# tudoroancea/ihm2

Hardware: AMD Instinct MI355X
Metric: NMPC RTI solves/s (batch), N=40, nx=8 (6-DOF bicycle), fkin6 (higher is better)
Workload: dtype f64

## Files before the change

ihm2_amd/csrc/device_steps.hpp:

```cpp
#pragma once

#include "ihm2mpc_internal.h"
#include "model.hpp"
#include "rk4.hpp"

namespace ihm2 {

__device__ __forceinline__ void dev_prepare(int b, int lane, int N, double s_target, int mode, const double *x0,
                                            double *x, double *u, double *yref, double *yref_e)
{
    double *xb = x + (size_t)b * (N + 1) * 8, *ub = u + (size_t)b * N * 2;
    if (mode & 1) {
        const double s0 = x0[(size_t)b * 8];
        double *yb = yref + (size_t)b * N * 12, *ye = yref_e + (size_t)b * 8;
        for (int e = lane; e < N * 12; e += 64) yb[e] = (e % 12 == 0) ? s0 + s_target * (e / 12) / N : 0.0;
        if (lane < 8) ye[lane] = (lane == 0) ? s0 + s_target : 0.0;
    }
    if (!(mode & 2)) return;
    const int nx = N * 8;
    for (int base = 0; base < nx; base += 64) {
        const int e = base + lane;
        const double v = (e < nx) ? xb[e + 8] : 0.0;
        __syncthreads();
        if (e < nx) xb[e] = v;
        __syncthreads();
    }
    const int nu = N * 2;
    for (int base = 0; base < nu; base += 64) {
        const int e = base + lane;
        const double v = (e < nu - 2) ? ub[e + 2] : 0.0;
        __syncthreads();
        if (e < nu) ub[e] = v;
        __syncthreads();
    }
}

__device__ __forceinline__ void dev_wrap_lap(int b, int lane, int N, int nknots, const double *__restrict__ s_ref, const int32_t *__restrict__ track_id,
                                             double *x0, double *x)
{
    const double L = -s_ref[(size_t)track_id[b] * nknots];
    if (!(x0[(size_t)b * 8] >= L)) return;
    for (int k = lane; k <= N; k += 64) x[((size_t)b * (N + 1) + k) * 8] -= L;
    if (lane == 0) x0[(size_t)b * 8] -= L;
}

__host__ __device__ constexpr int s_pos(int mdl, int c, int i)
{
    int p = 0;
    for (int cc = 0; cc < c; cc++)
        for (int b = 0; b < 8; b++) p += (S_COL_MASK[mdl][cc] >> b) & 1u;
    for (int b = 0; b < i; b++) p += (S_COL_MASK[mdl][c] >> b) & 1u;
    return p;
}
__host__ __device__ constexpr int s_count(int mdl) { return s_pos(mdl, 10, 0); }

template <int COL>
__device__ __forceinline__ double fkin6_factored_row(int i, const double (&J)[8][10], const double (&dX)[8], const double (&dK)[8])
{
    constexpr unsigned cm = S_COL_MASK[0][COL];
    double acc = 0.0;
    if (i == 2) {
        if ((cm >> 5) & 1u) acc = dX[5];
        acc = fma(-J[FKIN6_F_ROW2][FKIN6_F_DKS], dX[0], acc);
        acc = fma(-J[FKIN6_F_ROW2][FKIN6_F_KAP], dK[0], acc);
    } else {
        if (COL == 9) acc = -J[FKIN6_F_ROW5][FKIN6_F_DBD_DU];
        if ((cm >> 4) & 1u) acc = fma(k_lR, dK[4], acc);
        if ((cm >> 7) & 1u) acc = fma(-J[FKIN6_F_ROW5][FKIN6_F_DBD_DD], dX[7], acc);
    }
    return acc;
}

template <int MODEL, int COL, bool FACTORED = false>
__device__ __forceinline__ void sens_col_stage(const double (&J)[8][10], const double (&S)[8], const double *Sl, double (&Sacc)[8],
                                               double (&dK)[8], double ah, double wh)
{
    static_assert(!FACTORED || MODEL == IHM2MPC_MODEL_FKIN6, "the factored Jacobian is fkin6's");
    constexpr unsigned cm = S_COL_MASK[MODEL ? 1 : 0][COL];
    double dX[8];
#pragma unroll
    for (int l = 0; l < 8; l++)
        if ((cm >> l) & 1u) dX[l] = fma(ah, dK[l], Sl ? Sl[s_pos(MODEL ? 1 : 0, COL, l) * 64] : S[l]);
#pragma unroll
    for (int i = 0; i < 8; i++) {
        if (!((cm >> i) & 1u)) continue;
        if (FACTORED && (i == 2 || i == 5)) { dK[i] = fkin6_factored_row<COL>(i, J, dX, dK); continue; }
        double acc = 0.0;
        if (COL >= 8 && ((JU_MASK[MODEL ? 1 : 0][i] >> (COL - 8)) & 1u)) acc = J[i][COL];
#pragma unroll
        for (int l = 0; l < 8; l++)
            if (((JX_MASK[MODEL ? 1 : 0][i] & cm) >> l) & 1u) acc = fma(J[i][l], dX[l], acc);
        dK[i] = acc;
    }
#pragma unroll
    for (int i = 0; i < 8; i++)
        if ((cm >> i) & 1u) Sacc[i] = fma(wh, dK[i], Sacc[i]);
}

template <int MODEL, int COL>
__device__ __forceinline__ void sens_col_copy(const double (&src)[8], double (&dst)[8])
{
    constexpr unsigned cm = S_COL_MASK[MODEL ? 1 : 0][COL];
#pragma unroll
    for (int i = 0; i < 8; i++)
        if ((cm >> i) & 1u) dst[i] = src[i];
}

template <int COL, bool FACTORED = false>
__device__ __forceinline__ void sens_col_stage_lag(const double (&J)[8][10], const double (&S)[8], double (&Sacc)[8], double (&dK)[8], double ah,
                                                   double wh, double E_T, double E_d)
{
    constexpr unsigned cm = S_COL_MASK[0][COL];
    double dX[8];
#pragma unroll
    for (int l = 0; l < 6; l++)
        if ((cm >> l) & 1u) dX[l] = fma(ah, dK[l], S[l]);
    if ((cm >> 6) & 1u) dX[6] = (COL == 8) ? fma(E_T, S[6], 1.0 - E_T) : E_T * S[6];
// ... 272 lines not shown
```

ihm2_amd/csrc/kernels_qp.hip:

```cpp
#include <cstring>

#include "ihm2mpc_internal.h"
#include "device_steps.hpp"
#include "sqp_body.hpp"
#include "irk_body.hpp"
#include "riccati_mfma.hpp"
#include "sens_body.hpp"
#include "qp_lds.hpp"
#include "qp_mrows.hpp"
#include "qp_reduce.hpp"
#include "qp_div.hpp"
#include "qp_catalogue.hpp"
#include "wave_sync.hpp"

using namespace ihm2;

namespace {

#define INF_BOUND 1e20
#ifndef RIC_RING
#define RIC_RING 4
#endif
#ifndef SWEEP_RING
#define SWEEP_RING 4
// ... 154 lines not shown
    constexpr bool HL = CLS.hl, CL = CLS.cl;
    static_assert(qp_factor_inside(qp_lds(40, CLS), 40, NCK) && qp_factor_inside(qp_lds(2, CLS), 2, NCK), "factor stage / block reductions leave their LDS");
    static_assert(qp_sweeps_inside(qp_lds(40, CLS), 40, LEAN != 0, SWEEP_RING, SWEEP_DL) && (LEAN == 0 || qp_sweeps_inside(qp_lds(2, CLS), 2, true, SWEEP_RING, SWEEP_DL)),
                  "the sweeps' unclamped LDS prefetch leaves the block (the earlier form does below N = 4: api.hip refuses those launches)");
    static_assert(NW <= 4, "qp_factor_inside checks the block reductions for four waves");
    static_assert(FULL == 0 || qp_full_zeroes_kept(qp_lds(NF > 0 ? NF : 2, CLS), NF > 0 ? NF : 2), "a store of the factor sweep reaches gam or cf: the full slot form zeroes them once per solve");
#define LEN(id) qp_lds_len(id, N, NS, CLS)
    double *z = sm, *gt = z + LEN(QP_Z), *pi = gt + LEN(QP_GT), *pv = pi + LEN(QP_PI), *rb = pv + LEN(QP_PV), *gam = rb + LEN(QP_RB), *cf = gam + LEN(QP_GAM), *dz = cf + LEN(QP_CF);
    double *kff = dz + LEN(QP_DZ), *Kl = kff + LEN(QP_KFF), *Ginv = Kl + LEN(QP_KL), *Prb = Ginv + LEN(QP_GINV), *tile = Prb + LEN(QP_PRB), *hc = tile + LEN(QP_TILE), *ha = hc + LEN(QP_HC);
    double *Hl = ha + LEN(QP_HA), *CDl = Hl + LEN(QP_HL), *spv = CDl + LEN(QP_CDL);
    int *spc = reinterpret_cast<int *>(spv + 60);
#undef LEN
#define HS(k, i, l) (HL ? Hl[(((k) == N) ? 100 : 0) + (i) * 10 + (l)] : ((k) == N ? HsT : Hs0 + (UNI ? 0 : (k)) * 100)[(i) * 10 + (l)])
#define CDV(k, r, j) (CL ? CDl[(r) * 10 + (j)] : a.CD[((k) * 2 + (r)) * 10 + (j)])

    auto blk_reduce = [&](double v, auto op) -> double {
        v = wave_reduce(v, op);
        if (NW > 1) {
            __syncthreads();
            if (lane == 0) tile[wv] = v;
            __syncthreads();
            v = tile[0];
#pragma unroll
            for (int w = 1; w < NW; w++) v = op(v, tile[w]);
        }
        return v;
    };
    auto blk_max = [&](double v) { return blk_reduce(v, [](double x, double y) { return fmax(x, y); }); };
    auto blk_min = [&](double v) { return blk_reduce(v, [](double x, double y) { return fmin(x, y); }); };
    auto blk_sum = [&](double v) { return blk_reduce(v, [](double x, double y) { return x + y; }); };
    auto blk_nanmax = [&](double v) { return blk_reduce(v, [](double x, double y) { return nanmax(x, y); }); };

    const double *xb = a.x + (size_t)b * NS * 8;
    const double *ub = a.u + (size_t)b * N * 2;
    const double *linb = a.lin + (size_t)b * N * LIN_REC;
    double *gb = a.g + (size_t)b * NS * 10;
    double *rgb = a.rg + (size_t)b * NS * 10;
    double *Pg = a.P + (size_t)b * NS * 64;
    double *Mg = a.M + (size_t)b * N * 64;
    double *pib = a.pi + (size_t)b * NS * 8;
    double *lamb = a.lam + (size_t)b * NS * 28;
    double *slkb = a.slk + (size_t)b * NS * 28;
    double *lamab = ALAT ? a.lam_a + (size_t)b * NS * 2 : nullptr;
    double *slkab = ALAT ? a.slk_a + (size_t)b * NS * 2 : nullptr;
    auto alat_slot = [](int j) -> int { return (j == 3) ? 0 : (j == 4) ? 1 : (j == 6) ? 2 : (j == 7) ? 3 : -1; };

    if (HL) for (int e = tid; e < 200; e += NT) Hl[e] = (e < 100) ? Hs0[e] : HsT[e - 100];
    if (CL && tid < 20) CDl[tid] = a.CD[tid];
    if (UNI) BSYNC();
    bool h_sparse = false;
    if (HL) {
        int cnt = 0;
        if (tid < 20) {
#pragma unroll
            for (int l = 0; l < 10; l++) {
                const double v = Hl[tid * 10 + l];
                if (v != 0.0) { if (cnt < 3) { spv[tid * 3 + cnt] = v; spc[tid * 3 + cnt] = l; } cnt++; }
            }
            for (int q = cnt; q < 3; q++) { spv[tid * 3 + q] = 0.0; spc[tid * 3 + q] = 0; }
        }
        h_sparse = __ballot(cnt > 3) == 0ull;
        if (NW > 1) h_sparse = blk_max((wv == 0 && !h_sparse) ? 1.0 : 0.0) == 0.0;
        BSYNC();
    }
    double sg = 1.0, sb = 1.0, r_stat = 0.0, r_eq = 0.0;
    double w_R = 0.0, w_L = 0.0;
    if (PATH) {
        const int trk = a.track_id[b];
        w_R = a.widths[trk * 2 + 0]; w_L = a.widths[trk * 2 + 1];
        for (int k = tid; k < NS; k += NT) {
            const double psi = xb[k * 8 + 2], sgn = (psi > 0.0) - (psi < 0.0);
            const double dfoot = -0.5 * a.car_L * cos(fabs(psi)) * sgn, dlat = -0.5 * a.car_W * sin(psi);
            hc[k * 2 + 0] = (k >= 1) ? dfoot + dlat : 0.0;
            hc[k * 2 + 1] = (k >= 1) ? -dfoot + dlat : 0.0;
            if (ALAT) {
                double g4[4];
                alat_eval(xb[k * 8 + 3], xb[k * 8 + 4], xb[k * 8 + 6], xb[k * 8 + 7], g4);
#pragma unroll
                for (int q = 0; q < 4; q++) ha[k * 4 + q] = (k >= 1 && k < N) ? g4[q] : 0.0;
            }
        }
        BSYNC();
    }
    for (int e = tid; e < NS * 10; e += NT) {
        const int k = e / 10, j = e % 10;
        double acc = 0.0;
#pragma unroll
        for (int l = 0; l < 8; l++) acc = fma(HS(k, j, l), xb[k * 8 + l], acc);
        if (k < N) {
            acc = fma(HS(k, j, 8), ub[k * 2 + 0], acc);
            acc = fma(HS(k, j, 9), ub[k * 2 + 1], acc);
            const double *yr = a.yref + ((size_t)b * N + k) * 12;
#pragma unroll
            for (int l = 0; l < 12; l++) acc = fma(-Gy0[((UNI ? 0 : k) * 10 + j) * 12 + l], yr[l], acc);
        } else {
            const double *yr = a.yref_e + (size_t)b * 8;
#pragma unroll
            for (int l = 0; l < 8; l++) acc = fma(-GyT[j * 12 + l], yr[l], acc);
        }
        gb[e] = acc;
        const bool counted = !((k == 0 && j < 8) || (k == N && j >= 8));
        if (j < 8 || k < N) sg = fmax(sg, fabs(acc));
        if (!want_res) continue;
        double st = acc;
        if (k < N) {
            const double *rec = linb + (size_t)k * LIN_REC;
#pragma unroll
            for (int l = 0; l < 8; l++) st = fma((j < 8) ? rec[l * 8 + j] : rec[64 + l * 2 + (j - 8)], pib[(k + 1) * 8 + l], st);
        }
        if (j < 8) st -= pib[k * 8 + j];
        st -= lamb[k * 28 + j] - lamb[k * 28 + 14 + j];
        if (k < N) {
            st = fma(-CDV(k, 0, j), lamb[k * 28 + 10] - lamb[k * 28 + 24], st);
            st = fma(-CDV(k, 1, j), lamb[k * 28 + 11] - lamb[k * 28 + 25], st);
        }
        if (PATH && (j == 1 || j == 2)) {
            const double l12 = lamb[k * 28 + 12] - lamb[k * 28 + 26], l13 = lamb[k * 28 + 13] - lamb[k * 28 + 27];
            st -= (j == 1) ? l12 - l13 : hc[k * 2] * l12 + hc[k * 2 + 1] * l13;
        }
        if (ALAT && alat_slot(j) >= 0) st -= ha[k * 4 + alat_slot(j)] * (lamab[k * 2] - lamab[k * 2 + 1]);
        if (counted) r_stat = fmax(r_stat, fabs(st));
    }
    for (int e = tid; e < N * 8; e += NT) {
        const double bl = linb[(size_t)(e / 8) * LIN_REC + 80 + (e % 8)];
        sb = fmax(sb, fabs(bl));
        r_eq = fmax(r_eq, fabs(bl));
    }
    if (tid < 8) {
        const double d = a.x0[(size_t)b * 8 + tid] - xb[tid];
        sb = fmax(sb, fabs(d));
        r_eq = fmax(r_eq, fabs(d));
    }
    if constexpr (FULL != 0) { double sg2 = sg, sb2 = sb; wave_max4(lane, sg, sb, sg2, sb2); }
    else { sg = blk_max(sg); sb = blk_max(sb); }

    int s_kc[NSLOT];
    double s_dl[NSLOT], s_du[NSLOT];
    double lam_l[NSLOT], lam_u[NSLOT], t_l[NSLOT], t_u[NSLOT];
    constexpr int NSO = (NSOFT > 0) ? NSOFT : 1;
    double so_zw[NSO], so_Zw[NSO], so_s[NSO], so_ls[NSO], so_rs[NSO], so_ds[NSO], so_dls[NSO], so_pa[NSO];
#pragma unroll
    for (int r = 0; r < NSO; r++) { so_zw[r] = 0.0; so_Zw[r] = -1.0; so_s[r] = 1.0; so_ls[r] = 0.0; so_rs[r] = 0.0; so_ds[r] = so_dls[r] = so_pa[r] = 0.0; }
#define IS_SOFT(r) ((r) < NSOFT && so_Zw[(r) < NSOFT ? (r) : 0] >= 0.0)
#define ONE_SIDED(r) (NSOFT > 0 && PATH != 2 && (r) < NSOFT)
#define HAS_L(r) (FULL ? true : ONE_SIDED(r) ? true : fin(s_dl[r]))
#define HAS_U(r) (FULL ? true : ONE_SIDED(r) ? false : fin(s_du[r]))
#define ROW_DOT(r, v) (FULL ? row_dot_full((r), (v)) : ONE_SIDED(r) ? s_sg[(r) < NSOFT ? (r) : 0] * row_dot(s_kc[r], (v)) : row_dot(s_kc[r], (v)))
#define NO_SLOT(r) (!FULL && s_kc[r] < 0)
#define SLOT_W(r) (FULL ? (s_kc[r] & 0xffff) >> 3 : s_kc[r])
#define SLOT_AT(arr, r) (*(FULL ? reinterpret_cast<double *>(reinterpret_cast<char *>(arr) + (here(s_kc[r]) & 0xffff)) : &(arr)[s_kc[r]]))
#define ROW_SIGN(r, c) (ONE_SIDED(r) ? s_sg[(r) < NSOFT ? (r) : 0] * (c) : (c))
    double s_sg[NSO];
#pragma unroll
    for (int r = 0; r < NSO; r++) s_sg[r] = 1.0;
#define SLOT_ACC(dst, v) do { if (NSOFT > 0) (dst) += (v); else (dst) = (v); } while (0)
    double r_ineq = 0.0, r_comp = 0.0;
#pragma unroll
    for (int r = 0; r < NSLOT; r++) {
        const int s = tid + NT * r;
        s_kc[r] = FULL ? 0 : -1; s_dl[r] = -INFINITY; s_du[r] = INFINITY;
        lam_l[r] = lam_u[r] = 0.0; t_l[r] = t_u[r] = 1.0;
        const int kc = (s < a.nslots) ? a.slot_kc[s] : -1;
        if (kc >= 0) {
            const int k = kc >> 4, c = kc & 15;
            s_kc[r] = k * NCK + c;
            if (FULL) s_kc[r] = qp_full_slot_pack(k, c, NCK);
            double cz;
            if (c < 8) cz = xb[k * 8 + c];
            else if (c < 10) cz = ub[k * 2 + c - 8];
            else if (ALAT && c == 14) {
                double g4[4];
                cz = alat_eval(xb[k * 8 + 3], xb[k * 8 + 4], xb[k * 8 + 6], xb[k * 8 + 7], g4);
            } else if (c >= 12) {
                const double n = xb[k * 8 + 1], psi = xb[k * 8 + 2];
                const double foot = -0.5 * a.car_L * sin(fabs(psi)), lat = 0.5 * a.car_W * cos(psi);
                cz = (c == 12) ? n + foot + lat - w_R : -n - foot + lat - w_L;
            } else {
                cz = 0.0;
#pragma unroll
                for (int j = 0; j < 8; j++) cz = fma(CDV(k, c - 10, j), xb[k * 8 + j], cz);
                cz = fma(CDV(k, c - 10, 8), ub[k * 2 + 0], cz);
                cz = fma(CDV(k, c - 10, 9), ub[k * 2 + 1], cz);
            }
            const double lb = slot_lbb[s], ubd = slot_ubb[s];
            bool soft = false;
            if (r < NSOFT) { so_zw[r < NSOFT ? r : 0] = a.slot_zw[s]; so_Zw[r < NSOFT ? r : 0] = a.slot_Zw[s]; soft = a.slot_Zw[s] >= 0.0; }
#define LAM_IN(up) ((ALAT && c == 14) ? lamab[k * 2 + (up)] : lamb[k * 28 + 14 * (up) + c])
            if (fin(lb)) { s_dl[r] = lb - cz; if (want_res && !soft) { r_ineq = fmax(r_ineq, s_dl[r]); r_comp = fmax(r_comp, fabs(LAM_IN(0) * s_dl[r])); } }
            if (fin(ubd)) { s_du[r] = ubd - cz; if (want_res && !soft) { r_ineq = fmax(r_ineq, -s_du[r]); r_comp = fmax(r_comp, fabs(LAM_IN(1) * s_du[r])); } }
#undef LAM_IN
            if (ONE_SIDED(r) && fin(ubd)) { s_sg[r < NSOFT ? r : 0] = -1.0; s_dl[r] = -s_du[r]; }
        }
    }
    if (want_res) {
        if constexpr (FULL != 0) wave_max4(lane, r_stat, r_eq, r_ineq, r_comp);
        else { r_stat = blk_max(r_stat); r_eq = blk_max(r_eq); r_ineq = blk_max(r_ineq); r_comp = blk_max(r_comp); }
    }
    if (want_res && tid == 0) {
        double *rs = a.res + (size_t)b * 4;
        rs[0] = r_stat; rs[1] = r_eq; rs[2] = r_ineq; rs[3] = r_comp;
    }

    const double tol_g = a.tol * sg, tol_b = a.tol * sb, tol_d = a.tol * sb, tol_m = a.tol * sg;
    const double mu_floor = 0.1 * tol_m;
    const double mu0 = a.mu0 * sg;
    const double inv_m = (a.m_act > 0) ? 1.0 / a.m_act : 0.0;

    auto row_dot = [&](int kc, const double *v) -> double {
        const int k = kc / NCK, c = kc % NCK;
        if (c < 10) return v[k * 10 + c];
        if (ALAT && c == 14) return ha[k * 4] * v[k * 10 + 3] + ha[k * 4 + 1] * v[k * 10 + 4] + ha[k * 4 + 2] * v[k * 10 + 6] + ha[k * 4 + 3] * v[k * 10 + 7];
        if (PATH && c >= 12) return (c == 12) ? v[k * 10 + 1] + hc[k * 2] * v[k * 10 + 2] : -v[k * 10 + 1] + hc[k * 2 + 1] * v[k * 10 + 2];
        double acc = 0.0;
#pragma unroll
        for (int j = 0; j < 10; j++) acc = fma(CDV(k, c - 10, j), v[k * 10 + j], acc);
        return acc;
    };
    auto row_dot_full = [&](int r, const double *v) -> double {
        const int pk = here(s_kc[r]);
        return *reinterpret_cast<const double *>(reinterpret_cast<const char *>(pk < 0 ? tile : v) + ((pk >> 16) & 0x3fff));
    };
    static_assert(FULL == 0 || qp_general_rows_inside(qp_lds(NF > 0 ? NF : 2, CLS), NF > 0 ? NF : 2), "the general rows of a phase leave the transpose tile");
    auto general_rows = [&](const double *v) {
        for (int e0 = tid; e0 < 2 * N; e0 += 2 * NT) {
            const bool two = e0 + NT < 2 * N;
            const double *cd = CDl + (e0 & 1) * 10, *v0 = v + (e0 >> 1) * 10, *v1 = v + ((two ? e0 + NT : e0) >> 1) * 10;
            double c[10], p[10], q[10];
#pragma unroll
            for (int j = 0; j < 10; j++) { c[j] = cd[j]; p[j] = v0[j]; q[j] = v1[j]; }
            double acc0 = 0.0, acc1 = 0.0;
#pragma unroll
            for (int j = 0; j < 10; j++) { acc0 = fma(c[j], p[j], acc0); acc1 = fma(c[j], q[j], acc1); }
            tile[e0] = acc0;
            if (two) tile[e0 + NT] = acc1;
        }
        BSYNC();
    };

    for (int e = tid; e < NS * 10; e += NT) z[e] = (e < 8) ? a.x0[(size_t)b * 8 + e] - xb[e] : 0.0;
    for (int e = tid; e < NS * 8; e += NT) pi[e] = 0.0;
    if (FULL) for (int e = tid; e < NS * NCK; e += NT) { cf[e] = 0.0; gam[e] = 0.0; }
    BSYNC();
    if constexpr (FULL != 0) general_rows(z);
#pragma unroll
    for (int r = 0; r < NSLOT; r++) {
        if (NO_SLOT(r)) continue;
        const double rz = ROW_DOT(r, z);
        const bool al = HAS_L(r), au = HAS_U(r);
        double tau_c = a.tau0;
        if (al && au) tau_c = fmin(a.tau0, 0.25 * (s_du[r] - s_dl[r]));
        if (IS_SOFT(r)) {
            const double slack = al ? rz - s_dl[r] : s_du[r] - rz;
            const double s0 = fmax(a.tau0, a.tau0 - slack);
            so_s[r < NSOFT ? r : 0] = s0;
            so_ls[r < NSOFT ? r : 0] = mu0 / s0;
            if (al) { t_l[r] = slack + s0; lam_l[r] = mu0 / t_l[r]; } else { t_u[r] = slack + s0; lam_u[r] = mu0 / t_u[r]; }
            continue;
        }
        if (al) { t_l[r] = fmax(rz - s_dl[r], tau_c); lam_l[r] = mu0 / t_l[r]; }
        if (au) { t_u[r] = fmax(s_du[r] - rz, tau_c); lam_u[r] = mu0 / t_u[r]; }
    }

    int qstatus = 1, it = 0;
    bool exact_mode = false;
    double res_g = 0, res_b = 0, res_d = 0, res_m = 0, mu = 0;
    double fol_g = 0.0, fol_b = 0.0;
    double rd_l[NSLOT], rd_u[NSLOT], dlam_l[NSLOT], dlam_u[NSLOT], dt_l[NSLOT], dt_u[NSLOT];
// ... 16 lines not shown
        if (LEAN != 0) { if (exact) multipliers_to_cf(); }
        else {
            for (int e = tid; e < NS * NCK; e += NT) cf[e] = 0.0;
            BSYNC();
        }
        double mu_acc = 0.0, res_gs = 0.0;
        res_d = 0.0; res_m = 0.0;
        double lane_d = 0.0, lane_m = 0.0;
        bool bad_d = false, bad_m = false, bad_gs = false;
        if constexpr (FULL != 0) general_rows(z);
#pragma unroll
        for (int r = 0; r < NSLOT; r++) {
            rd_l[r] = rd_u[r] = 0.0;
            if (NO_SLOT(r)) continue;
            const double rz = ROW_DOT(r, z);
            const bool al = HAS_L(r), au = HAS_U(r);
            const double sv = IS_SOFT(r) ? so_s[r < NSOFT ? r : 0] : 0.0;
            double pl = 0.0, pu = 0.0;
            if constexpr (FULL != 0) {
                rd_l[r] = rz - t_l[r] - s_dl[r] + sv; pl = __dmul_rn(lam_l[r], t_l[r]); norm_max(lane_m, bad_m, fabs(pl));
                rd_u[r] = s_du[r] - rz - t_u[r] + sv; pu = __dmul_rn(lam_u[r], t_u[r]); norm_max(lane_m, bad_m, fabs(pu));
            } else {
            if (al) { rd_l[r] = rz - t_l[r] - s_dl[r] + sv; pl = __dmul_rn(lam_l[r], t_l[r]); res_m = nanmax(res_m, fabs(pl)); }
            if (au) { rd_u[r] = s_du[r] - rz - t_u[r] + sv; pu = __dmul_rn(lam_u[r], t_u[r]); res_m = nanmax(res_m, fabs(pu)); }
            }
            mu_acc = __dadd_rn(mu_acc, __dadd_rn(pl, pu));
            if constexpr (FULL != 0) { bad_d |= __builtin_isunordered(rd_l[r], rd_u[r]); lane_d = fmax(lane_d, fmax(fabs(rd_l[r]), fabs(rd_u[r]))); }
            else
            res_d = nanmax(res_d, nanmax(fabs(rd_l[r]), fabs(rd_u[r])));
            if (IS_SOFT(r)) {
                const int q = r < NSOFT ? r : 0;
                so_rs[q] = so_Zw[q] * so_s[q] + so_zw[q] - (al ? lam_l[r] : lam_u[r]) - so_ls[q];
                if constexpr (FULL != 0) {
                    norm_max(res_gs, bad_gs, fabs(so_rs[q]));
                    mu_acc += so_ls[q] * so_s[q]; norm_max(lane_m, bad_m, fabs(so_ls[q] * so_s[q]));
                } else {
                res_gs = nanmax(res_gs, fabs(so_rs[q]));
                mu_acc += so_ls[q] * so_s[q]; res_m = nanmax(res_m, fabs(so_ls[q] * so_s[q]));
                }
            }
            if (LEAN == 0) SLOT_ACC(SLOT_AT(cf, r), ROW_SIGN(r, (al ? lam_l[r] : 0.0) - (au ? lam_u[r] : 0.0)));
        }
        if constexpr (NW > 1) {
#pragma unroll
            for (int r = 0; r < NSLOT; r++) {
                const int sidx = tid + NT * r;
                if (sidx >= a.nslots_can) continue;
                const bool on = s_kc[r] >= 0;
                gam[sidx] = __dadd_rn((on && fin(s_dl[r])) ? __dmul_rn(lam_l[r], t_l[r]) : 0.0, (on && fin(s_du[r])) ? __dmul_rn(lam_u[r], t_u[r]) : 0.0);
            }
            __syncthreads();
            mu_acc = 0.0;
            for (int sidx = lane; sidx < a.nslots_can; sidx += 64) mu_acc = __dadd_rn(mu_acc, gam[sidx]);
            __syncthreads();
        }
        if (LEAN == 0) BSYNC();
        for (int rpass = 0; rpass < 2; rpass++) {
            if (exact) {
                for (int e = tid; e < NS * 10; e += NT) {
                    const int k = e / 10, j = e % 10;
                    double acc = gb[e];
                    if (HL && h_sparse) {
                        const int row = ((k == N) ? 10 : 0) + j;
#pragma unroll
                        for (int q = 0; q < 3; q++) acc = fma(spv[row * 3 + q], z[k * 10 + spc[row * 3 + q]], acc);
                    } else {
#pragma unroll
                        for (int l = 0; l < 10; l++) acc = fma(HS(k, j, l), z[k * 10 + l], acc);
                    }
                    if (k < N) {
                        acc = fma(-CDV(k, 0, j), cf[k * NCK + 10], acc);
                        acc = fma(-CDV(k, 1, j), cf[k * NCK + 11], acc);
                    }
                    if (j < 8) acc -= pi[k * 8 + j];
                    acc -= cf[k * NCK + j];
                    if (PATH && (j == 1 || j == 2)) {
                        const double l12 = cf[k * NCK + 12], l13 = cf[k * NCK + 13];
                        acc -= (j == 1) ? l12 - l13 : hc[k * 2] * l12 + hc[k * 2 + 1] * l13;
                    }
                    if (ALAT && alat_slot(j) >= 0) acc -= ha[k * 4 + alat_slot(j)] * cf[k * NCK + 14];
                    gt[e] = acc;
                }
                BSYNC();
                dyn_residual<4, NT>(N, tid, const_cast<double *>(linb), z, pi, gt, rb, LIN_REC);
                BSYNC();
            }
            res_g = 0.0; res_b = 0.0;
            if (exact || LEAN == 0) {
                for (int e = tid; e < NS * 10; e += NT) {
                    const int k = e / 10, j = e % 10;
                    double v = gt[e];
                    if ((k == 0 && j < 8) || (k == N && j >= 8)) { v = 0.0; gt[e] = 0.0; }
                    if (exact) rgb[e] = v;
                    res_g = nanmax(res_g, fabs(v));
                }
                for (int e = tid; e < N * 8; e += NT) res_b = nanmax(res_b, fabs(rb[e]));
            } else { res_g = fol_g; res_b = fol_b; }
            if constexpr (FULL != 0) {
                const bool nan_g = wave_any(res_g != res_g || bad_gs), nan_b = wave_any(res_b != res_b), nan_d = wave_any(bad_d), nan_m = wave_any(bad_m);
                res_g = fmax(res_g, res_gs);
                res_d = lane_d; res_m = lane_m;
                wave_max4(lane, res_g, res_b, res_d, res_m);
                mu = wave_sum(mu_acc) * inv_m;
                res_g = nan_g ? NAN : res_g; res_b = nan_b ? NAN : res_b; res_d = nan_d ? NAN : res_d; res_m = nan_m ? NAN : res_m;
            } else {
            res_g = nanmax(res_g, res_gs);
            res_g = blk_nanmax(res_g); res_b = blk_nanmax(res_b);
            if (rpass == 0) { res_d = blk_nanmax(res_d); res_m = blk_nanmax(res_m); mu = ((NW == 1) ? blk_sum(mu_acc) : wave_sum(mu_acc)) * inv_m; }
            }
            if (!(res_g == res_g) || !(res_b == res_b) || !(res_d == res_d) || !(res_m == res_m)) { qstatus = (it == 0) ? 3 : 4; finished = true; break; }
            const bool conv = res_g <= tol_g && res_b <= tol_b && res_d <= tol_d && res_m <= tol_m;
            if (conv && exact) { qstatus = 0; finished = true; break; }
            if ((conv || it >= a.iter_max) && !exact) {
                exact = true; exact_mode = true;
                if (LEAN != 0) multipliers_to_cf();
                continue;
            }
            break;
        }
        if (finished) break;
        if (it >= a.iter_max) { qstatus = 1; break; }
        BSYNC();
        double alpha = 1.0, alpha_d = 1.0, sigma = 0.0;
        auto slot_coeffs = [&](int pass) {
            if (!FULL) {
                for (int e = tid; e < NS * NCK; e += NT) { cf[e] = 0.0; if (pass == 0) gam[e] = 0.0; }
                BSYNC();
            }
            const double mu_t = fmax(sigma * mu, mu_floor);
            if constexpr (FULL != 0) {
                if (pass == 1) {
                    double cn[2 * NSLOT], cd[2 * NSLOT], cq[2 * NSLOT];
#pragma unroll
                    for (int r = 0; r < NSLOT; r++) { cn[2 * r] = pa_l[r] - mu_t; cd[2 * r] = t_l[r]; cn[2 * r + 1] = pa_u[r] - mu_t; cd[2 * r + 1] = t_u[r]; }
                    div_sets<DIVW_COEFF>(cn, cd, cq);
#pragma unroll
                    for (int r = 0; r < NSLOT; r++) {
                        double c = 0.0;
                        c += cq[2 * r];
                        c -= cq[2 * r + 1];
                        SLOT_AT(cf, r) = c;
                    }
                    BSYNC();
                    return;
                }
            }
#pragma unroll
            for (int r = 0; r < NSLOT; r++) {
                if (NO_SLOT(r)) continue;
                const bool al = HAS_L(r), au = HAS_U(r);
                double c = 0.0;
                if (IS_SOFT(r)) {
                    const int q = r < NSOFT ? r : 0;
                    const double lm = al ? lam_l[r] : lam_u[r], tt = al ? t_l[r] : t_u[r], rdv = al ? rd_l[r] : rd_u[r];
                    const double gm = lm / tt, gs = so_ls[q] / so_s[q], D = so_Zw[q] + gm + gs;
                    double c1, c2, rsv;
                    if (pass == 0) { c1 = (lm * tt + lm * rdv) / tt; c2 = so_ls[q]; rsv = so_rs[q]; SLOT_AT(gam, r) += gm * (so_Zw[q] + gs) / D; }
                    else { c1 = ((al ? pa_l[r] : pa_u[r]) - mu_t) / tt; c2 = (so_pa[q] - mu_t) / so_s[q]; rsv = 0.0; }
                    c = c1 - gm * (rsv + c1 + c2) / D;
                    SLOT_AT(cf, r) += ONE_SIDED(r) ? ROW_SIGN(r, c) : (al ? c : -c);
                    continue;
                }
                if (pass == 0) {
                    const double gl = al ? lam_l[r] / t_l[r] : 0.0, gu = au ? lam_u[r] / t_u[r] : 0.0;
                    if (al) c += fma(gl, rd_l[r], lam_l[r]);
                    if (au) c -= fma(gu, rd_u[r], lam_u[r]);
// ... 471 lines not shown
    irk_linearize_quad<MODEL>(st, rows, x + ((size_t)b * (N + 1) + k) * 8, u + ((size_t)b * N + k) * 2, tid, nknots, s_ref, kappa_ref,
                              lin + ((size_t)b * N + k) * LIN_REC, q < N);
}
__device__ __noinline__ void call_sim_step(int b, int q, int model, int M, double dt, int nknots, const double *s_ref, const double *kappa_ref,
                                           const int32_t *track_id, const double *xs, const double *us, double *xn)
{
    dev_sim_step(b, q, model, M, dt, nknots, s_ref, kappa_ref, track_id, xs, us, xn, nullptr);
}

__device__ __noinline__ void call_sim_irk(const IrkTab *tab, int b, int model, int M, int nknots, const double *s_ref, const double *kappa_ref,
                                          const int32_t *track_id, const double *u0, double *x0)
{
    const int st = threadIdx.x & 3;
    double x[8];
#pragma unroll
    for (int a = 0; a < 8; a++) x[a] = x0[(size_t)b * 8 + a];
    const double u_T = u0[(size_t)b * 2], u_d = u0[(size_t)b * 2 + 1];
    const int tid = track_id[b];
    TrackSeg trk;
    trk.init(s_ref + (size_t)tid * nknots, kappa_ref + (size_t)tid * nknots, nknots, x[0]);
    const IrkRows rows = irk_rows_from(tab, st);
    irk_sim_quad(st, rows, model, M, x, u_T, u_d, trk);
    __syncthreads();
    if (threadIdx.x == 0)
#pragma unroll
        for (int a = 0; a < 8; a++) x0[(size_t)b * 8 + a] = x[a];
}

template <int MODEL, bool ROLL>
__device__ __noinline__ void call_line_search(const LsArgs &ls, int b, int it, int last)
{
    line_search_body<MODEL, ROLL>(ls, b, it, last);
}

template <int NSLOT, int NSOFT, int PATH, int UNI, int SQP, int IRK = 0, int DYN = 0, int SENS = 0, int NF = 0, int FULL = 0>
__global__ __launch_bounds__(64) void k_steps(const StepArgs *sp, QpArgs a, const LsArgs *lsp)
{
    static_assert(DYN == 0 || s_count(1) == QP_DYN_RK4_WORDS, "the dynamic models' RK4 integrator parks s_count(1) words per lane in the QP's LDS (qp_lds.hpp: steps_lds_doubles)");
    const StepArgs &s = *sp;
    const LsArgs &ls = *lsp;
    extern __shared__ double sm[];
    const int b = blockIdx.x, lane = threadIdx.x;
    if (b >= a.B) return;
    if (NF > 0 && a.N != NF) return;
    const int N = (NF > 0) ? NF : a.N;
    const size_t B = a.B;
    auto stop_from = [&](int step) {
        if (s.active && lane == 0) s.active[b] = 0;
        for (int t = step; t < s.n_steps; t++) {
            if (s.hist_u0 && lane < 2) s.hist_u0[((size_t)t * B + b) * 2 + lane] = 0.0;
            if (s.hist_x0 && lane < 8) s.hist_x0[((size_t)t * B + b) * 8 + lane] = s.x0[(size_t)b * 8 + lane];
            if (s.hist_st && lane == 0) s.hist_st[(size_t)t * B + b] = a.status[b];
            if (s.hist_it && lane == 0) s.hist_it[(size_t)t * B + b] = 0;
        }
        if constexpr (SENS != 0) {
            const SensArgs &sa = *s.sens;
            const int NS = N + 1;
            if (sa.hist && lane < 16)
                for (int t = step; t < s.n_steps; t++) sa.hist[((size_t)t * B + b) * 16 + lane] = NAN;
            if (lane < 16) sa.sens_u0[(size_t)b * 16 + lane] = NAN;
            if (sa.mode == 2) {
                for (int e = lane; e < NS * 64; e += 64) sa.sens_x[(size_t)b * NS * 64 + e] = NAN;
                for (int e = lane; e < N * 16; e += 64) sa.sens_u[(size_t)b * N * 16 + e] = NAN;
            }
        }
    };
    for (int step = 0; step < s.n_steps; step++) {
        bool act = s.active ? s.active[b] != 0 : true;
        if (s.freeze && act) {
            const int st = a.status[b];
            if (st != 0 && st != 2) act = false;
        }
        if (!act && s.freeze) { stop_from(step); return; }
        if (s.lap_wrap) { dev_wrap_lap(b, lane, N, s.nknots, s.s_ref, a.track_id, s.x0, a.x); __syncthreads(); }
        const double x_old = (lane < 8) ? s.x0[(size_t)b * 8 + lane] : 0.0;
        const bool irk_plant = s.sim_irk_tab != nullptr;
        const bool kin_plant = (IRK == 2 ? s.sim_lag != 0 : !IRK) && !irk_plant && s.model == IHM2MPC_MODEL_FKIN6;
        double *spare = s.lin + (size_t)B * N * LIN_REC;
        if (!kin_plant && act) {
            if (irk_plant) call_sim_irk(s.sim_irk_tab, b, s.model, s.M_sim, s.nknots, s.s_ref, s.kappa_ref, a.track_id, a.u0, s.x0);
            else if (lane < 4) call_sim_step(b, lane, s.model, s.M_sim, s.dt, s.nknots, s.s_ref, s.kappa_ref, a.track_id, s.x0, a.u0, s.x0);
            __syncthreads();
        }
        dev_prepare(b, lane, N, s.s_target, 2, s.x0, a.x, a.u, s.yref, s.yref_e);
        const int n_it = SQP ? s.sqp_iters : 1;
        if (SQP && lane == 0) { ls.done[b] = 0; ls.sqp_iter[b] = 0; ls.qp_acc[b] = 0; }
        __syncthreads();
        for (int it = 0; it < n_it; it++) {
            if (SQP) {
                const int NS = N + 1;
                for (int e = lane; e < NS * 8; e += 64) {
                    ((double *)ls.xp)[(size_t)b * NS * 8 + e] = a.x[(size_t)b * NS * 8 + e];
                    ((double *)ls.pip)[(size_t)b * NS * 8 + e] = a.pi[(size_t)b * NS * 8 + e];
                }
                for (int e = lane; e < N * 2; e += 64) ((double *)ls.up)[(size_t)b * N * 2 + e] = a.u[(size_t)b * N * 2 + e];
                for (int e = lane; e < NS * 28; e += 64) {
                    ((double *)ls.lamp)[(size_t)b * NS * 28 + e] = a.lam[(size_t)b * NS * 28 + e];
                    ((double *)ls.slkp)[(size_t)b * NS * 28 + e] = a.slk[(size_t)b * NS * 28 + e];
                }
            }
            {
                const int tid = a.track_id[b];
                const bool with_plant = kin_plant && it == 0 && act;
                const int om = DYN ? s.ocp_model : IHM2MPC_MODEL_FKIN6;
                if (IRK == 1) {
                    for (int base = 0; base < N; base += 16) {
                        if constexpr (!DYN) call_linearize_irk<IHM2MPC_MODEL_FKIN6>(s.irk_tab, b, base, N, s.nknots, s.s_ref, s.kappa_ref, tid, a.x, a.u, s.lin);
                        else {
                            if (om == IHM2MPC_MODEL_FDYN6U) call_linearize_irk<IHM2MPC_MODEL_FDYN6U>(s.irk_tab, b, base, N, s.nknots, s.s_ref, s.kappa_ref, tid, a.x, a.u, s.lin);
                            else call_linearize_irk<IHM2MPC_MODEL_FDYN6>(s.irk_tab, b, base, N, s.nknots, s.s_ref, s.kappa_ref, tid, a.x, a.u, s.lin);
                        }
                    }
                } else
                for (int k = lane; k < N + (with_plant ? 1 : 0); k += 64) {
                    const bool plant = k == N;
                    const double *xk = plant ? s.x0 + (size_t)b * 8 : a.x + ((size_t)b * (N + 1) + k) * 8;
                    const double *uk = plant ? a.u0 + (size_t)b * 2 : a.u + ((size_t)b * N + k) * 2;
                    double *rec = plant ? spare + (size_t)b * LIN_REC : s.lin + ((size_t)b * N + k) * LIN_REC;
                    if constexpr (IRK == 2)
                        call_integrate_fkin6_lag(xk, uk, plant ? xk : xk + 8, tid, plant ? s.M_sim : s.M, s.dt, s.nknots, s.s_ref, s.kappa_ref, rec,
                                                 plant ? s.x0 + (size_t)b * 8 : nullptr, s.lag[plant ? 1 : 0]);
                    else if (!DYN || plant)
                        call_integrate_fkin6(xk, uk, plant ? xk : xk + 8, tid, plant ? s.M_sim : s.M, s.dt, s.nknots, s.s_ref, s.kappa_ref, rec,
                                             plant ? s.x0 + (size_t)b * 8 : nullptr);
                    else if constexpr (DYN != 0) {
                        if (om == IHM2MPC_MODEL_FDYN6U)
                            call_integrate_dyn<IHM2MPC_MODEL_FDYN6U>(xk, uk, xk + 8, tid, s.M, s.dt, s.nknots, s.s_ref, s.kappa_ref, rec, sm + lane);
                        else
                            call_integrate_dyn<IHM2MPC_MODEL_FDYN6>(xk, uk, xk + 8, tid, s.M, s.dt, s.nknots, s.s_ref, s.kappa_ref, rec, sm + lane);
                    }
                }
            }
            __syncthreads();
            if constexpr (SENS != 0) {
                const SensArgs &sa = *s.sens;
                const int NS = N + 1;
                for (int e = lane; e < NS * 8; e += 64) ((double *)sa.xbar)[(size_t)b * NS * 8 + e] = a.x[(size_t)b * NS * 8 + e];
                for (int e = lane; e < N * 2; e += 64) ((double *)sa.ubar)[(size_t)b * N * 2 + e] = a.u[(size_t)b * N * 2 + e];
            }
            if (it == 0) {
                if (s.freeze) {
                    const double v = (lane < 8) ? s.x0[(size_t)b * 8 + lane] : 0.0;
                    if (__any(v != v)) {
                        if (lane < 8) s.x0[(size_t)b * 8 + lane] = x_old;
                        __syncthreads();
                        stop_from(step);
                        return;
                    }
                }
                dev_prepare(b, lane, N, s.s_target, 1, s.x0, a.x, a.u, s.yref, s.yref_e);
                __syncthreads();
            }
            qp_wave_body<NSLOT, NSOFT, PATH, UNI, 1, SQP ? 0 : 1, NF, FULL>(a, b, sm, SQP || step + 1 == s.n_steps);
            __syncthreads();
            if constexpr (SENS != 0) {
                sens_body(*s.sens, b, sm, step);
                __syncthreads();
            }
            if (SQP) {
                const int last = it == n_it - 1;
                if constexpr (!DYN) call_line_search<IHM2MPC_MODEL_FKIN6, IRK != 0>(ls, b, it, last);
                else {
                    if (s.ocp_model == IHM2MPC_MODEL_FDYN6U) call_line_search<IHM2MPC_MODEL_FDYN6U, IRK != 0>(ls, b, it, last);
                    else call_line_search<IHM2MPC_MODEL_FDYN6, IRK != 0>(ls, b, it, last);
                }
                __syncthreads();
            }
// ... 27 lines not shown
```

ihm2_amd/csrc/riccati_mfma.hpp:

```cpp
#pragma once
#ifdef RIC_STAMPS
__device__ long long ric_dbg[8];
#define RIC_STAMP_DECL long long ric_T[8] = {0, 0, 0, 0, 0, 0, 0, 0}, ric_tp = __builtin_readcyclecounter(); int ric_cur = 7;
#define RIC_STAMP(i) do { const long long t_now = __builtin_readcyclecounter(); ric_T[ric_cur] += t_now - ric_tp; ric_tp = t_now; ric_cur = (i); } while (0)
#define RIC_STAMP_OUT do { if (threadIdx.x == 0 && blockIdx.x == 0) for (int q = 0; q < 8; q++) ric_dbg[q] = ric_T[q]; } while (0)
#else
#define RIC_STAMP_DECL
#define RIC_STAMP(i)
#define RIC_STAMP_OUT
#endif

#include <hip/hip_runtime.h>

#include "qp_lds.hpp"
#include "qp_mrows.hpp"
#include "wave_sync.hpp"

namespace ihm2 {

typedef double d4_t __attribute__((ext_vector_type(4)));
#define IHM2_MFMA_F64(a, b, c) __builtin_amdgcn_mfma_f64_16x16x4f64((a), (b), (c), 0, 0, 0)

template <int CTRL>
__device__ __forceinline__ double dpp_mov(double v)
{
    int lo = __double2loint(v), hi = __double2hiint(v);
    lo = __builtin_amdgcn_mov_dpp(lo, CTRL, 0xF, 0xF, false);
    hi = __builtin_amdgcn_mov_dpp(hi, CTRL, 0xF, 0xF, false);
    return __hiloint2double(hi, lo);
}
__device__ __forceinline__ double readlane_f64(double v, int lane)
{
    return __hiloint2double(__builtin_amdgcn_readlane(__double2hiint(v), lane), __builtin_amdgcn_readlane(__double2loint(v), lane));
}

#define RIC_IDX(row, col) (((((row) & 3) * 8 + (col)) << 1) + ((row) >> 2))
#define RIC_REC_RB 88

struct RicLds {
    int gam;
    int hc;
    int ha;
    int gt;
    int pv;
    int hv;
    int Kl;
    int Ginv;
    int kff;
    int dz;
    int tile;
};

template <int NB, int NT = 64>
__device__ __forceinline__ void dyn_residual(const int N, const int lane, double *linb, const double *z, const double *pi, double *gt, double *rb,
                                             const int lin_rec)
{
    const int n1 = N * 8;
    for (int base = 0; base < n1; base += NT * NB) {
        double2 Ar[NB][4], Br[NB];
        double br[NB];
#pragma unroll
        for (int q = 0; q < NB; q++) {
            const int e = min(base + NT * q + lane, n1 - 1), k = e >> 3, o = e & 7;
            const double *rec = linb + (size_t)k * lin_rec;
            const double2 *row = reinterpret_cast<const double2 *>(rec + o * 8);
#pragma unroll
            for (int l = 0; l < 4; l++) Ar[q][l] = row[l];
            Br[q] = *reinterpret_cast<const double2 *>(rec + 64 + o * 2);
            br[q] = rec[80 + o];
        }
#pragma unroll
        for (int q = 0; q < NB; q++) {
            const int e = base + NT * q + lane, ec = min(e, n1 - 1), k = ec >> 3, o = ec & 7;
            double acc = br[q] - z[(k + 1) * 10 + o];
#pragma unroll
            for (int l = 0; l < 4; l++) { acc = fma(Ar[q][l].x, z[k * 10 + 2 * l], acc); acc = fma(Ar[q][l].y, z[k * 10 + 2 * l + 1], acc); }
            acc = fma(Br[q].x, z[k * 10 + 8], acc);
            acc = fma(Br[q].y, z[k * 10 + 9], acc);
            if (e < n1) {
                rb[e] = acc;
                linb[(size_t)k * lin_rec + RIC_REC_RB + o] = acc;
            }
        }
    }
    const int n2 = N * 10;
    for (int base = 0; base < n2; base += NT * NB) {
        double cr[NB][8];
#pragma unroll
        for (int q = 0; q < NB; q++) {
            const int e = min(base + NT * q + lane, n2 - 1), k = e / 10, jz = e - k * 10;
            const double *rec = linb + (size_t)k * lin_rec;
            const double *col = (jz < 8) ? rec + jz : rec + 64 + (jz - 8);
            const int cs = (jz < 8) ? 8 : 2;
#pragma unroll
            for (int l = 0; l < 8; l++) cr[q][l] = col[l * cs];
        }
#pragma unroll
        for (int q = 0; q < NB; q++) {
            const int e = base + NT * q + lane, ec = min(e, n2 - 1), k = ec / 10;
            double acc = gt[ec];
#pragma unroll
            for (int l = 0; l < 8; l++) acc = fma(cr[q][l], pi[(k + 1) * 8 + l], acc);
            if (e < n2) gt[e] = acc;
        }
    }
}

template <int NCK, bool PATH, bool UNI, int D, bool ALAT = false, bool PLAIN = false, int NF = 0>
__device__ __forceinline__ void riccati_sweep_mfma(const int N_rt, const int lane, const double *__restrict__ linb, const double *__restrict__ Hs,
                                                   const double *__restrict__ HsT,
                                                   const double *__restrict__ CD, const RicLds L, double *__restrict__ Pg, double *__restrict__ Mg,
                                                   const int lin_rec, const bool store_p, const bool symmetrize)
{
    static_assert(!PLAIN || (UNI && !PATH && !ALAT), "the straight-line stage is written for the batch-shared all-hard tables");
    static_assert(PLAIN || NF == 0, "a compile-time horizon comes with the straight-line stage");
    const int N = (NF > 0) ? NF : N_rt;
    const int g = lane >> 4, j = lane & 15;
    const int col = (j < 10) ? j : (j == 12) ? 9 : (j == 13) ? 8 : -1;
    const int row[4] = {g, g + 4, (g < 2) ? 8 + g : -1, (g == 0) ? 9 : (g == 1) ? 8 : -1};
    const double m10 = (j == 10) ? 1.0 : 0.0;
    extern __shared__ double ric_sm[];
#define sm ric_sm

    unsigned off[2], offB;
#pragma unroll
    for (int c = 0; c < 2; c++) {
        const int rr = 4 * c + g;
        off[c] = (j < 8) ? rr * 8 + j : (col >= 0) ? 64 + rr * 2 + (col - 8) : RIC_REC_RB + rr;
    }
    offB = (j >= 8) ? 64 + (j - 8) * 2 + (g & 1) : 0;
    double hconst[4], cc0[4], cc1[4], dsel[4];
    int va[4], vstride[4];
#pragma unroll
    for (int r = 0; r < 4; r++) {
        const bool ok = row[r] >= 0 && col >= 0, gr = row[r] >= 0 && j == 10;
        hconst[r] = (UNI && ok) ? Hs[row[r] * 10 + col] : 0.0;
        cc0[r] = (UNI && ok) ? CD[row[r]] * CD[col] : 0.0;
        cc1[r] = (UNI && ok) ? CD[10 + row[r]] * CD[10 + col] : 0.0;
        dsel[r] = ((ok && row[r] == col) || gr) ? 1.0 : 0.0;
        vstride[r] = (j == 10) ? 10 : NCK;
        va[r] = ((j == 10) ? L.gt : L.gam) + ((r == 3) ? ((row[3] >= 0) ? row[3] : 0) : g) + (N - 1) * vstride[r];
    }
    int a_g10 = L.gam + (N - 1) * NCK + 10;
    const double p11 = (PATH && row[0] == 1 && col == 1) ? 1.0 : 0.0, p22 = (PATH && row[0] == 2 && col == 2) ? 1.0 : 0.0;
    const double p12 = (PATH && ((row[0] == 1 && col == 2) || (row[0] == 2 && col == 1))) ? 1.0 : 0.0;
    auto a_slot = [](int c) -> int { return (c == 3) ? 0 : (c == 4) ? 1 : (c == 6) ? 2 : (c == 7) ? 3 : -1; };
    const int as_c = ALAT ? a_slot(col) : -1, as_r0 = ALAT ? a_slot(row[0]) : -1, as_r1 = ALAT ? a_slot(row[1]) : -1;
    const double am0 = (as_c >= 0 && as_r0 >= 0) ? 1.0 : 0.0, am1 = (as_c >= 0 && as_r1 >= 0) ? 1.0 : 0.0;
    const int ao_c = L.ha + max(as_c, 0), ao_r0 = L.ha + max(as_r0, 0), ao_r1 = L.ha + max(as_r1, 0);
    const double selA0 = (g == 0) ? 1.0 : 0.0, selA2 = (g == 1) ? 1.0 : 0.0, selB = (g < 2) ? -1.0 : 0.0;

    const int a_tw = L.tile + g * QP_TILE_ROW + j, a_tr = L.tile + (j & 7) * QP_TILE_ROW + g;
    const double wS = (j < 8) ? 0.5 : 1.0, wT = (j < 8) ? 0.5 : 0.0;

    d4_t Pd;
    {
        const double g12 = PATH ? sm[L.gam + N * NCK + 12] : 0.0, g13 = PATH ? sm[L.gam + N * NCK + 13] : 0.0;
        const double a0 = PATH ? sm[L.hc + N * 2] : 0.0, a1 = PATH ? sm[L.hc + N * 2 + 1] : 0.0;
#pragma unroll
        for (int r = 0; r < 2; r++) {
            double v = 0.0;
            if (j < 8) {
                v = HsT[row[r] * 10 + j];
                if (row[r] == j) v += sm[L.gam + N * NCK + j];
            } else if (j == 10) v = sm[L.gt + N * 10 + row[r]];
            if (PATH && r == 0) v += p11 * (g12 + g13) + p12 * (g12 * a0 - g13 * a1) + p22 * (g12 * a0 * a0 + g13 * a1 * a1);
            Pd[r] = v;
            if (j < 8) Pg[(size_t)N * 64 + RIC_IDX(row[r], j)] = v;
            if (j == 10) sm[L.pv + N * 8 + row[r]] = v;
        }
        Pd[2] = Pd[3] = 0.0;
    }

    double r0[D], r1[D], rB[D];
    const int rec_bytes = lin_rec * 8;
    const __amdgpu_buffer_rsrc_t rsrc = __builtin_amdgcn_make_buffer_rsrc(const_cast<double *>(linb), 0, PLAIN ? N * rec_bytes : 0, 0x00020000);
    const unsigned vo0 = off[0] * 8u, vo1 = off[1] * 8u, voB = offB * 8u;
    typedef unsigned int ric_u2_t __attribute__((ext_vector_type(2)));
    auto rec_load = [&](const unsigned voff, const int soff) -> double {
        const ric_u2_t v = __builtin_amdgcn_raw_buffer_load_b64(rsrc, voff, soff, 0);
        return __hiloint2double((int)v.y, (int)v.x);
    };
#pragma unroll
    for (int d = 0; d < D; d++) {
        if constexpr (PLAIN) {
            const int so = max(N - 1 - d, 0) * rec_bytes;
// ... 156 lines not shown
```

Baseline: 1.389 million.

## Batch loads in gradient, slot setup, and shift; specialize first-iteration dynamics residual

In the FULL (compile-time horizon) path, the gradient loop now loads the x, u, yref and Gy operands for two entries into registers before computing, and the equality-residual loop becomes a fully unrolled register batch. Slot setup prefetches slot_kc, bounds and the primal values up front, and the horizon shift runs with one pair of barriers instead of one pair per chunk. A specialized first-iteration dynamics residual reuses the already-loaded linearisation offsets and only computes the k=0 product, assuming the other stages are zero when the offsets are finite. These changes aim to overlap memory latency and cut barriers, at the cost of more registers and reliance on the first-iteration primal being zero beyond the first stage.

```diff
diff --git a/ihm2_amd/csrc/device_steps.hpp b/ihm2_amd/csrc/device_steps.hpp
--- a/ihm2_amd/csrc/device_steps.hpp
+++ b/ihm2_amd/csrc/device_steps.hpp
@@ -33,6 +33,24 @@
         if (e < nu) ub[e] = v;
         __syncthreads();
     }
+}
+
+template <int HZN>
+__device__ __forceinline__ void dev_prepare_shift(int b, int lane, double *x, double *u)
+{
+    constexpr int nx = HZN * 8, nu = HZN * 2, CX = (nx + 63) / 64, CU = (nu + 63) / 64;
+    double *xb = x + (size_t)b * (HZN + 1) * 8, *ub = u + (size_t)b * HZN * 2;
+    double vx[CX], vu[CU];
+#pragma unroll
+    for (int c = 0; c < CX; c++) { const int e = c * 64 + lane; vx[c] = (e < nx) ? xb[e + 8] : 0.0; }
+#pragma unroll
+    for (int c = 0; c < CU; c++) { const int e = c * 64 + lane; vu[c] = (e < nu - 2) ? ub[e + 2] : 0.0; }
+    __syncthreads();
+#pragma unroll
+    for (int c = 0; c < CX; c++) { const int e = c * 64 + lane; if (e < nx) xb[e] = vx[c]; }
+#pragma unroll
+    for (int c = 0; c < CU; c++) { const int e = c * 64 + lane; if (e < nu) ub[e] = vu[c]; }
+    __syncthreads();
 }
 
 __device__ __forceinline__ void dev_wrap_lap(int b, int lane, int N, int nknots, const double *__restrict__ s_ref, const int32_t *__restrict__ track_id,
diff --git a/ihm2_amd/csrc/kernels_qp.hip b/ihm2_amd/csrc/kernels_qp.hip
--- a/ihm2_amd/csrc/kernels_qp.hip
+++ b/ihm2_amd/csrc/kernels_qp.hip
@@ -260,6 +260,66 @@
         }
         BSYNC();
     }
+#define GRAD_ENTRY_TAIL \
+        gb[e] = acc; \
+        const bool counted = !((k == 0 && j < 8) || (k == N && j >= 8)); \
+        if (j < 8 || k < N) sg = fmax(sg, fabs(acc)); \
+        if (!want_res) continue; \
+        double st = acc; \
+        if (k < N) { \
+            const double *rec = linb + (size_t)k * LIN_REC; \
+        _Pragma("unroll") \
+            for (int l = 0; l < 8; l++) st = fma((j < 8) ? rec[l * 8 + j] : rec[64 + l * 2 + (j - 8)], pib[(k + 1) * 8 + l], st); \
+        } \
+        if (j < 8) st -= pib[k * 8 + j]; \
+        st -= lamb[k * 28 + j] - lamb[k * 28 + 14 + j]; \
+        if (k < N) { \
+            st = fma(-CDV(k, 0, j), lamb[k * 28 + 10] - lamb[k * 28 + 24], st); \
+            st = fma(-CDV(k, 1, j), lamb[k * 28 + 11] - lamb[k * 28 + 25], st); \
+        } \
+        if (PATH && (j == 1 || j == 2)) { \
+            const double l12 = lamb[k * 28 + 12] - lamb[k * 28 + 26], l13 = lamb[k * 28 + 13] - lamb[k * 28 + 27]; \
+            st -= (j == 1) ? l12 - l13 : hc[k * 2] * l12 + hc[k * 2 + 1] * l13; \
+        } \
+        if (ALAT && alat_slot(j) >= 0) st -= ha[k * 4 + alat_slot(j)] * (lamab[k * 2] - lamab[k * 2 + 1]); \
+        if (counted) r_stat = fmax(r_stat, fabs(st));
+    if constexpr (FULL != 0) {
+        constexpr int GRAD_B = 2, n10 = (NF + 1) * 10;
+        for (int e0 = tid; e0 < n10; e0 += NT * GRAD_B) {
+            double xo[GRAD_B][10], yo[GRAD_B][12], go[GRAD_B][12];
+#pragma unroll
+            for (int q = 0; q < GRAD_B; q++) {
+                const int e = min(e0 + NT * q, n10 - 1), k = e / 10, j = e % 10;
+                const bool mid = k < N;
+                const double *yr = mid ? a.yref + ((size_t)b * N + k) * 12 : a.yref_e + (size_t)b * 8;
+                const double *gy = mid ? Gy0 + j * 12 : GyT + j * 12;
+#pragma unroll
+                for (int l = 0; l < 8; l++) { xo[q][l] = xb[k * 8 + l]; yo[q][l] = yr[l]; go[q][l] = gy[l]; }
+#pragma unroll
+                for (int l = 8; l < 12; l++) { yo[q][l] = mid ? yr[l] : 0.0; go[q][l] = mid ? gy[l] : 0.0; }
+                xo[q][8] = mid ? ub[k * 2 + 0] : 0.0;
+                xo[q][9] = mid ? ub[k * 2 + 1] : 0.0;
+            }
+#pragma unroll
+            for (int q = 0; q < GRAD_B; q++) {
+                const int e = e0 + NT * q, ec = min(e, n10 - 1), k = ec / 10, j = ec % 10;
+                double acc = 0.0;
+#pragma unroll
+                for (int l = 0; l < 8; l++) acc = fma(HS(k, j, l), xo[q][l], acc);
+                if (k < N) {
+                    acc = fma(HS(k, j, 8), xo[q][8], acc);
+                    acc = fma(HS(k, j, 9), xo[q][9], acc);
+#pragma unroll
+                    for (int l = 0; l < 12; l++) acc = fma(-go[q][l], yo[q][l], acc);
+                } else {
+#pragma unroll
+                    for (int l = 0; l < 8; l++) acc = fma(-go[q][l], yo[q][l], acc);
+                }
+                if (e >= n10) continue;
+                GRAD_ENTRY_TAIL
+            }
+        }
+    } else
     for (int e = tid; e < NS * 10; e += NT) {
         const int k = e / 10, j = e % 10;
         double acc = 0.0;
@@ -276,29 +336,23 @@
 #pragma unroll
             for (int l = 0; l < 8; l++) acc = fma(-GyT[j * 12 + l], yr[l], acc);
         }
-        gb[e] = acc;
-        const bool counted = !((k == 0 && j < 8) || (k == N && j >= 8));
-        if (j < 8 || k < N) sg = fmax(sg, fabs(acc));
-        if (!want_res) continue;
-        double st = acc;
-        if (k < N) {
-            const double *rec = linb + (size_t)k * LIN_REC;
-#pragma unroll
-            for (int l = 0; l < 8; l++) st = fma((j < 8) ? rec[l * 8 + j] : rec[64 + l * 2 + (j - 8)], pib[(k + 1) * 8 + l], st);
-        }
-        if (j < 8) st -= pib[k * 8 + j];
-        st -= lamb[k * 28 + j] - lamb[k * 28 + 14 + j];
-        if (k < N) {
-            st = fma(-CDV(k, 0, j), lamb[k * 28 + 10] - lamb[k * 28 + 24], st);
-            st = fma(-CDV(k, 1, j), lamb[k * 28 + 11] - lamb[k * 28 + 25], st);
-        }
-        if (PATH && (j == 1 || j == 2)) {
-            const double l12 = lamb[k * 28 + 12] - lamb[k * 28 + 26], l13 = lamb[k * 28 + 13] - lamb[k * 28 + 27];
-            st -= (j == 1) ? l12 - l13 : hc[k * 2] * l12 + hc[k * 2 + 1] * l13;
-        }
-        if (ALAT && alat_slot(j) >= 0) st -= ha[k * 4 + alat_slot(j)] * (lamab[k * 2] - lamab[k * 2 + 1]);
-        if (counted) r_stat = fmax(r_stat, fabs(st));
-    }
+        GRAD_ENTRY_TAIL
+    }
+#undef GRAD_ENTRY_TAIL
+    [[maybe_unused]] bool b_finite = true;
+    if constexpr (FULL != 0) {
+        constexpr int n8 = NF * 8, NR = (n8 + NT - 1) / NT;
+        double bl[NR];
+#pragma unroll
+        for (int q = 0; q < NR; q++) { const int e = min(tid + NT * q, n8 - 1); bl[q] = linb[(size_t)(e / 8) * LIN_REC + 80 + (e % 8)]; }
+#pragma unroll
+        for (int q = 0; q < NR; q++)
+            if (tid + NT * q < n8) { sb = fmax(sb, fabs(bl[q])); r_eq = fmax(r_eq, fabs(bl[q])); }
+        bool bad = false;
+#pragma unroll
+        for (int q = 0; q < NR; q++) bad |= !isfinite(bl[q]);
+        b_finite = !__any(bad);
+    } else
     for (int e = tid; e < N * 8; e += NT) {
         const double bl = linb[(size_t)(e / 8) * LIN_REC + 80 + (e % 8)];
         sb = fmax(sb, fabs(bl));
@@ -333,19 +387,36 @@
     for (int r = 0; r < NSO; r++) s_sg[r] = 1.0;
 #define SLOT_ACC(dst, v) do { if (NSOFT > 0) (dst) += (v); else (dst) = (v); } while (0)
     double r_ineq = 0.0, r_comp = 0.0;
+    [[maybe_unused]] int kc_pre[FULL ? NSLOT : 1];
+    [[maybe_unused]] double lb_pre[FULL ? NSLOT : 1], ub_pre[FULL ? NSLOT : 1], cz_pre[FULL ? NSLOT : 1];
+    if constexpr (FULL != 0) {
+#pragma unroll
+        for (int r = 0; r < NSLOT; r++) {
+            const int s = tid + NT * r;
+            const bool in = s < a.nslots;
+            kc_pre[r] = in ? a.slot_kc[s] : -1;
+            lb_pre[r] = in ? slot_lbb[s] : 0.0;
+            ub_pre[r] = in ? slot_ubb[s] : 0.0;
+        }
+#pragma unroll
+        for (int r = 0; r < NSLOT; r++) {
+            const int kc = max(kc_pre[r], 0), k = kc >> 4, c = kc & 15;
+            cz_pre[r] = (c < 8) ? xb[k * 8 + c] : ub[min(k, N - 1) * 2 + ((c < 10) ? c - 8 : 0)];
+        }
+    }
 #pragma unroll
     for (int r = 0; r < NSLOT; r++) {
         const int s = tid + NT * r;
         s_kc[r] = FULL ? 0 : -1; s_dl[r] = -INFINITY; s_du[r] = INFINITY;
         lam_l[r] = lam_u[r] = 0.0; t_l[r] = t_u[r] = 1.0;
-        const int kc = (s < a.nslots) ? a.slot_kc[s] : -1;
+        const int kc = FULL ? kc_pre[FULL ? r : 0] : (s < a.nslots) ? a.slot_kc[s] : -1;
         if (kc >= 0) {
             const int k = kc >> 4, c = kc & 15;
             s_kc[r] = k * NCK + c;
             if (FULL) s_kc[r] = qp_full_slot_pack(k, c, NCK);
             double cz;
-            if (c < 8) cz = xb[k * 8 + c];
-            else if (c < 10) cz = ub[k * 2 + c - 8];
+            if (c < 8) cz = FULL ? cz_pre[FULL ? r : 0] : xb[k * 8 + c];
+            else if (c < 10) cz = FULL ? cz_pre[FULL ? r : 0] : ub[k * 2 + c - 8];
             else if (ALAT && c == 14) {
                 double g4[4];
                 cz = alat_eval(xb[k * 8 + 3], xb[k * 8 + 4], xb[k * 8 + 6], xb[k * 8 + 7], g4);
@@ -360,7 +431,7 @@
                 cz = fma(CDV(k, c - 10, 8), ub[k * 2 + 0], cz);
                 cz = fma(CDV(k, c - 10, 9), ub[k * 2 + 1], cz);
             }
-            const double lb = slot_lbb[s], ubd = slot_ubb[s];
+            const double lb = FULL ? lb_pre[FULL ? r : 0] : slot_lbb[s], ubd = FULL ? ub_pre[FULL ? r : 0] : slot_ubb[s];
             bool soft = false;
             if (r < NSOFT) { so_zw[r < NSOFT ? r : 0] = a.slot_zw[s]; so_Zw[r < NSOFT ? r : 0] = a.slot_Zw[s]; soft = a.slot_Zw[s] >= 0.0; }
 #define LAM_IN(up) ((ALAT && c == 14) ? lamab[k * 2 + (up)] : lamb[k * 28 + 14 * (up) + c])
@@ -543,6 +614,10 @@
                     gt[e] = acc;
                 }
                 BSYNC();
+                if constexpr (FULL != 0) {
+                    if (it == 0 && b_finite) dyn_residual_first<NF>(tid, const_cast<double *>(linb), z, rb, LIN_REC);
+                    else dyn_residual<4, NT>(N, tid, const_cast<double *>(linb), z, pi, gt, rb, LIN_REC);
+                } else
                 dyn_residual<4, NT>(N, tid, const_cast<double *>(linb), z, pi, gt, rb, LIN_REC);
                 BSYNC();
             }
@@ -1180,7 +1255,8 @@
             else if (lane < 4) call_sim_step(b, lane, s.model, s.M_sim, s.dt, s.nknots, s.s_ref, s.kappa_ref, a.track_id, s.x0, a.u0, s.x0);
             __syncthreads();
         }
-        dev_prepare(b, lane, N, s.s_target, 2, s.x0, a.x, a.u, s.yref, s.yref_e);
+        if constexpr (FULL != 0) dev_prepare_shift<NF>(b, lane, a.x, a.u);
+        else dev_prepare(b, lane, N, s.s_target, 2, s.x0, a.x, a.u, s.yref, s.yref_e);
         const int n_it = SQP ? s.sqp_iters : 1;
         if (SQP && lane == 0) { ls.done[b] = 0; ls.sqp_iter[b] = 0; ls.qp_acc[b] = 0; }
         __syncthreads();
diff --git a/ihm2_amd/csrc/riccati_mfma.hpp b/ihm2_amd/csrc/riccati_mfma.hpp
--- a/ihm2_amd/csrc/riccati_mfma.hpp
+++ b/ihm2_amd/csrc/riccati_mfma.hpp
@@ -102,6 +102,42 @@
 #pragma unroll
             for (int l = 0; l < 8; l++) acc = fma(cr[q][l], pi[(k + 1) * 8 + l], acc);
             if (e < n2) gt[e] = acc;
+        }
+    }
+}
+
+template <int NF>
+__device__ __forceinline__ void dyn_residual_first(const int lane, double *linb, const double *z, double *rb, const int lin_rec)
+{
+    constexpr int n1 = NF * 8, NR = (n1 + 63) / 64;
+    double br[NR];
+#pragma unroll
+    for (int q = 0; q < NR; q++) {
+        const int e = min(64 * q + lane, n1 - 1);
+        br[q] = linb[(size_t)(e >> 3) * lin_rec + 80 + (e & 7)];
+    }
+    double2 Ar[4], Br;
+    {
+        const int o = lane & 7;
+        const double2 *row = reinterpret_cast<const double2 *>(linb + o * 8);
+#pragma unroll
+        for (int l = 0; l < 4; l++) Ar[l] = row[l];
+        Br = *reinterpret_cast<const double2 *>(linb + 64 + o * 2);
+    }
+    if (lane < 8) {
+        double acc = br[0] - z[10 + lane];
+#pragma unroll
+        for (int l = 0; l < 4; l++) { acc = fma(Ar[l].x, z[2 * l], acc); acc = fma(Ar[l].y, z[2 * l + 1], acc); }
+        acc = fma(Br.x, z[8], acc);
+        acc = fma(Br.y, z[9], acc);
+        br[0] = acc;
+    }
+#pragma unroll
+    for (int q = 0; q < NR; q++) {
+        const int e = 64 * q + lane;
+        if (e < n1) {
+            rb[e] = br[q];
+            linb[(size_t)(e >> 3) * lin_rec + RIC_REC_RB + (e & 7)] = br[q];
         }
     }
 }
```

New measurement: 1.395 million, median of 6. No clear change (+0.5%).
